# yutongwangBIT/multi_orbslam3

Measured on AMD Instinct MI355X. Metric: tracking+localBA frames/sec (aggregate over agents; 1 agent per GPU), higher is better.
Workload: dtype u8/int32 (ORB front-end, Hamming), f64 (local BA)

## Files before the change

### multi_orbslam3_amd/csrc/lba.hip

```cpp

#include <time.h>

#include <condition_variable>
#include <atomic>
#include <unistd.h>
#include <mutex>
#include <thread>

#include "common.hpp"
#include "wave.hpp"

#include <algorithm>
#include <cmath>
#include <limits>
#include <numeric>
#include <type_traits>

using namespace orbg;

#include "ldlt_mfma.hpp"
#include "ldlt_xcd.hpp"
#include "se3.hpp"
#include "lm_driver.hpp"

// ... 20 lines not shown
struct HostRec { double chi2, scale, maxdiag, chi2_init; int ok; unsigned seq; unsigned long long c_chi2, c_scale, c_ok; };
__host__ __device__ inline unsigned long long rec_tag(unsigned seq) { return (0x9E3779B97F4A7C15ull * ((unsigned long long)seq + 1ull)) | 1ull; }

template <class CamT>
__global__ __launch_bounds__(256) void k_export(int n_edges, int n_poses, int n_points, const lba_edge* __restrict__ edges,
                                               const PoseQ* __restrict__ poses, const double* __restrict__ points, CamT cam,
                                               const double* __restrict__ chi2, uint8_t* __restrict__ out_flags,
                                               double* __restrict__ out_chi2, PoseQ* __restrict__ out_poses,
                                               double* __restrict__ out_points) {
  const int k = blockIdx.x * 256 + threadIdx.x;
  if (k < n_edges) {
    const lba_edge e = edges[k];
    const bool depth_pos = edge_depth_positive(poses[e.pose], points + 3 * (size_t)e.point, cam, e);
    const double thr = e.ur < 0 ? 5.991 : 7.815;
    const double c = chi2[k];
    const bool outlier = c > thr || !depth_pos;
    out_flags[k] = (uint8_t)((depth_pos ? 1 : 0) | (outlier ? 2 : 0));
    if (out_chi2) out_chi2[k] = c;
  }
  if (k < n_poses) out_poses[k] = poses[k];
  if (k < 3 * n_points) out_points[k] = points[k];
}

struct LmIn { double cur_chi, lambda; const double* chi_p; const double* lambda_p; double* lambda_next; };

__device__ __forceinline__ void publish_trial_tail(int n_edge_blocks, const double* __restrict__ partial, unsigned* __restrict__ ticket,
                                                   const double* __restrict__ scale_partial, int n_scale_partial,
                                                   const int* __restrict__ ok_flag, HostRec* __restrict__ rec, unsigned seq, const LmIn lm,
                                                   int ok_override = 1) {
  __shared__ double parts[1024];
  const int np = n_edge_blocks;
  const int tot = min(np + n_scale_partial, 1024);
  for (int i = threadIdx.x; i < tot; i += 256)
    parts[i] = __hip_atomic_load(i < np ? &partial[i] : &scale_partial[i - np], __ATOMIC_RELAXED, __HIP_MEMORY_SCOPE_AGENT);
  __syncthreads();
  if (threadIdx.x == 0) {
    auto ordered_sum = [&](int first, int count) {
      double acc = 0;
      int i = 0;
      for (; i + 16 <= count; i += 16) {
        double v[16];
#pragma unroll
        for (int u = 0; u < 16; u++) v[u] = parts[first + i + u];
#pragma unroll
        for (int u = 0; u < 16; u++) acc += v[u];
      }
      for (; i < count; i++) acc += parts[first + i];
      return acc;
    };
    const int np_l = min(np, 1024), ns_l = max(min(np + n_scale_partial, 1024) - np_l, 0);
    double chi = ordered_sum(0, np_l), scale = ordered_sum(np_l, ns_l);
    for (int i = np_l; i < np; i++) chi += __hip_atomic_load(&partial[i], __ATOMIC_RELAXED, __HIP_MEMORY_SCOPE_AGENT);
    for (int i = ns_l; i < n_scale_partial; i++) scale += __hip_atomic_load(&scale_partial[i], __ATOMIC_RELAXED, __HIP_MEMORY_SCOPE_AGENT);
    const int okv = ok_override != 1 ? ok_override : ok_flag ? *ok_flag : 1;
    {
      const unsigned long long tg = rec_tag(seq), bc = (unsigned long long)__double_as_longlong(chi), bs = (unsigned long long)__double_as_longlong(scale);
      unsigned long long* r64 = reinterpret_cast<unsigned long long*>(rec);
      __hip_atomic_store(r64 + 0, bc, __ATOMIC_RELAXED, __HIP_MEMORY_SCOPE_SYSTEM);
      __hip_atomic_store(r64 + 1, bs, __ATOMIC_RELAXED, __HIP_MEMORY_SCOPE_SYSTEM);
      __hip_atomic_store(&rec->ok, okv, __ATOMIC_RELAXED, __HIP_MEMORY_SCOPE_SYSTEM);
      __hip_atomic_store(&rec->c_chi2, bc ^ tg, __ATOMIC_RELAXED, __HIP_MEMORY_SCOPE_SYSTEM);
      __hip_atomic_store(&rec->c_scale, bs ^ tg, __ATOMIC_RELAXED, __HIP_MEMORY_SCOPE_SYSTEM);
      __hip_atomic_store(&rec->c_ok, (unsigned long long)(unsigned)okv ^ tg, __ATOMIC_RELAXED, __HIP_MEMORY_SCOPE_SYSTEM);
    }
    if (lm.lambda_next) {
      const double cur = lm.chi_p ? *lm.chi_p : lm.cur_chi;
      const double lam = lm.lambda_p ? *lm.lambda_p : lm.lambda;
      const double tempChi = okv ? chi : 1.7976931348623157e308;
      double rho = cur - tempChi;
      rho /= scale + 1e-3;
      const double c3 = 2 * rho - 1;
      double alpha = 1. - c3 * c3 * c3;
      alpha = fmin(alpha, 2. / 3.);
      *lm.lambda_next = lam * fmax(1. / 3., alpha);
    }
    *ticket = 0;
    __hip_atomic_store(&rec->seq, seq, __ATOMIC_RELAXED, __HIP_MEMORY_SCOPE_SYSTEM);
  }
}
__device__ __forceinline__ unsigned trial_arrive(unsigned* __restrict__ ticket) {
  __builtin_amdgcn_fence(__ATOMIC_RELEASE, "agent");
  asm volatile("s_waitcnt vmcnt(0)" ::: "memory");
  return __hip_atomic_fetch_add(ticket, 1u, __ATOMIC_RELAXED, __HIP_MEMORY_SCOPE_AGENT);
}
__device__ __forceinline__ void publish_trial_record(int n_edge_blocks, const double* __restrict__ partial, unsigned* __restrict__ ticket,
                                                     const double* __restrict__ scale_partial, int n_scale_partial,
                                                     const int* __restrict__ ok_flag, HostRec* __restrict__ rec, unsigned seq,
                                                     const LmIn lm = LmIn{0, 0, nullptr, nullptr, nullptr}) {
  __shared__ int s_last;
  if (threadIdx.x == 0) s_last = (trial_arrive(ticket) == (unsigned)n_edge_blocks - 1);
  __syncthreads();
  if (!s_last) return;
  if (threadIdx.x == 0) {
    __builtin_amdgcn_fence(__ATOMIC_ACQUIRE, "agent");
    asm volatile("s_waitcnt vmcnt(0)" ::: "memory");
  }
  __syncthreads();
  publish_trial_tail(n_edge_blocks, partial, ticket, scale_partial, n_scale_partial, ok_flag, rec, seq, lm);
}
constexpr int kOkPublishTimedOut = -3;
__device__ __forceinline__ void publish_trial_when_all_arrived(int n_edge_blocks, const double* __restrict__ partial, unsigned* __restrict__ ticket,
                                                               const double* __restrict__ scale_partial, int n_scale_partial,
                                                               const int* __restrict__ ok_flag, HostRec* __restrict__ rec, unsigned seq, const LmIn lm) {
  __shared__ int s_ok;
  if (threadIdx.x == 0) {
    const long long t0 = (long long)wall_clock64();
    int ok = 1;
    for (unsigned polls = 0;; polls++) {
      if (__hip_atomic_load(ticket, __ATOMIC_RELAXED, __HIP_MEMORY_SCOPE_AGENT) >= (unsigned)n_edge_blocks) break;
      __builtin_amdgcn_s_sleep(1);
      if ((polls & 1023u) == 1023u && (long long)wall_clock64() - t0 > 200000000ll) { ok = kOkPublishTimedOut; break; }
    }
    s_ok = ok;
  }
  __syncthreads();
  publish_trial_tail(n_edge_blocks, partial, ticket, scale_partial, n_scale_partial, ok_flag, rec, seq, lm, s_ok);
}

template <class CamT>
__device__ __forceinline__ double errors_block(int bid, int n_edge_blocks, int n_edges, const lba_edge* __restrict__ edges,
                                               const PoseQ* __restrict__ poses, const double* __restrict__ points, CamT cam, Huber hb,
                                               double* __restrict__ err, double* __restrict__ chi2, double* __restrict__ partial,
                                               int final_mode, unsigned* __restrict__ ticket, const double* __restrict__ scale_partial,
                                               int n_scale_partial, const int* __restrict__ ok_flag, HostRec* __restrict__ rec,
                                               unsigned seq) {
  __shared__ double red[256];
  const int k = bid * 256 + threadIdx.x;
  double c_out = 0;
  double rho0 = 0;
  if (k < n_edges) {
    const lba_edge e = edges[k];
    double er[3], Xc[3];
    edge_error(poses[e.pose], points + 3 * (size_t)e.point, cam, e, er, Xc);
    const double om = (double)e.inv_sigma2;
    const int D = e.ur < 0 ? 2 : 3;
    double c = 0;
    for (int i = 0; i < D; i++) c += er[i] * (om * er[i]);
    err[3 * (size_t)k] = er[0]; err[3 * (size_t)k + 1] = er[1]; err[3 * (size_t)k + 2] = er[2];
    chi2[k] = c;
// ... 180 lines not shown
#pragma unroll
        for (int i = 0; i < 18; i++) out[i] = 0.0;
      } else if (pose_col[e.pose] >= 0 && point_col[e.point] >= 0) {
        for (int k2 = k + 1; k2 < n_edges; k2++) {
          const lba_edge e2 = edges[k2];
          if (e2.pose != e.pose || e2.point != e.point) break;
          double H2[18];
          edge_hpl<FUSED>(T, X, c, hb, e2, k2, err, chi2, H2);
#pragma unroll
          for (int i = 0; i < 18; i++) out[i] += H2[i];
        }
      }
    }
  }
  __syncthreads();
  const int valid = min(256, n_edges - bid * 256);
  double* dst = EB + (size_t)bid * 256 * kEB;
  for (int i = threadIdx.x; i < valid * kEB; i += 256) dst[i] = stage[i];
}
template <bool FUSED, class CamT>
__device__ __forceinline__ void lin_poses_block(int bid, const int* __restrict__ ps_start, const int* __restrict__ ps_edges,
                                                  const lba_edge* __restrict__ edges, const PoseQ* __restrict__ poses,
                                                  const double* __restrict__ points, CamT c, Huber hb, const double* __restrict__ err,
                                                  const double* __restrict__ chi2, double* __restrict__ Hpp, double* __restrict__ bp) {
  __shared__ double wpart[4][27];
  const int p = bid;
  const int b = ps_start[p], e_end = ps_start[p + 1];
  double acc[27];
#pragma unroll
  for (int i = 0; i < 27; i++) acc[i] = 0;
  constexpr int kCh = 3;
  for (int j0 = b + threadIdx.x; j0 < e_end; j0 += 256 * kCh) {
    int kk[kCh];
#pragma unroll
    for (int u = 0; u < kCh; u++) kk[u] = ps_edges[min(j0 + 256 * u, e_end - 1)];
    lba_edge ev[kCh];
#pragma unroll
    for (int u = 0; u < kCh; u++) ev[u] = edges[kk[u]];
    double Xv[kCh][3];
#pragma unroll
    for (int u = 0; u < kCh; u++) {
      const double* Xp = points + 3 * (size_t)ev[u].point;
      Xv[u][0] = Xp[0]; Xv[u][1] = Xp[1]; Xv[u][2] = Xp[2];
    }
    const PoseQ T = poses[ev[0].pose];
#pragma unroll
    for (int u = 0; u < kCh; u++) {
// ... 36 lines not shown
          acc[o++] += h;
        }
#pragma unroll
      for (int a = 0; a < 6; a++) {
        double sacc = 0;
#pragma unroll
        for (int i = 0; i < 3; i++) sacc += B[6 * i + a] * omega_r[i];
        acc[o++] += sacc;
      }
    }
  }
  const int lane = threadIdx.x & 63, wave = threadIdx.x >> 6;
#pragma unroll
  for (int i = 0; i < 27; i++) {
    const double v = wave_sum_f64(acc[i]);
    if (lane == 0) wpart[wave][i] = v;
  }
  __syncthreads();
  if (threadIdx.x < 27) {
    const double v = ((wpart[0][threadIdx.x] + wpart[1][threadIdx.x]) + wpart[2][threadIdx.x]) + wpart[3][threadIdx.x];
    if (threadIdx.x < 21) Hpp[21 * (size_t)p + threadIdx.x] = v;
    else bp[6 * (size_t)p + threadIdx.x - 21] = v;
  }
}


__device__ __forceinline__ double quad_get(double v, int src ) {
  int lo, hi;
  if (src == 1) { lo = __builtin_amdgcn_update_dpp(0, __double2loint(v), 0x55, 0xF, 0xF, true); hi = __builtin_amdgcn_update_dpp(0, __double2hiint(v), 0x55, 0xF, 0xF, true); }
  else if (src == 2) { lo = __builtin_amdgcn_update_dpp(0, __double2loint(v), 0xAA, 0xF, 0xF, true); hi = __builtin_amdgcn_update_dpp(0, __double2hiint(v), 0xAA, 0xF, 0xF, true); }
  else { lo = __builtin_amdgcn_update_dpp(0, __double2loint(v), 0xFF, 0xF, 0xF, true); hi = __builtin_amdgcn_update_dpp(0, __double2hiint(v), 0xFF, 0xF, 0xF, true); }
  return __hiloint2double(hi, lo);
}
template <class CamT>
__device__ __forceinline__ void lin_points_block(int bid, int nL, const int* __restrict__ pt_start, const int* __restrict__ pt_edges,
                                                   const lba_edge* __restrict__ edges, const PoseQ* __restrict__ poses,
                                                   const double* __restrict__ points, CamT c, Huber hb, double* __restrict__ Hll,
                                                   double* __restrict__ bl) {
  const int t = bid * 256 + threadIdx.x;
  const int l = min(t >> 2, nL - 1), q = t & 3;
  const bool mine = (t >> 2) < nL;
  double acc[9];
#pragma unroll
  for (int i = 0; i < 9; i++) acc[i] = 0;
  const int jb = pt_start[l], je = pt_start[l + 1];
  for (int j0 = jb + q; j0 < je; j0 += 8) {
    int id[2];
#pragma unroll
    for (int u = 0; u < 2; u++) id[u] = pt_edges[min(j0 + 4 * u, je - 1)];
    lba_edge ev[2];
#pragma unroll
    for (int u = 0; u < 2; u++) ev[u] = edges[id[u]];
    PoseQ Tv[2];
#pragma unroll
    for (int u = 0; u < 2; u++) Tv[u] = poses[ev[u].pose];
    const double* X = points + 3 * (size_t)ev[0].point;
    const double Xl[3] = {X[0], X[1], X[2]};
#pragma unroll
    for (int u = 0; u < 2; u++)
      if (j0 + 4 * u < je) {
        const lba_edge e = ev[u];
// ... 20 lines not shown
        for (int a = 0; a < 3; a++)
#pragma unroll
          for (int b2 = a; b2 < 3; b2++) {
            double h = 0;
#pragma unroll
            for (int i = 0; i < 3; i++) h += A[3 * i + a] * wom * A[3 * i + b2];
            acc[o++] += h;
          }
#pragma unroll
        for (int a = 0; a < 3; a++) {
          double sacc = 0;
#pragma unroll
          for (int i = 0; i < 3; i++) sacc += A[3 * i + a] * omega_r[i];
          acc[o++] += sacc;
        }
      }
  }
#pragma unroll
  for (int i = 0; i < 9; i++) acc[i] = ((acc[i] + quad_get(acc[i], 1)) + quad_get(acc[i], 2)) + quad_get(acc[i], 3);
  if (mine && q == 0) {
    for (int i = 0; i < 6; i++) Hll[6 * (size_t)l + i] = acc[i];
    for (int i = 0; i < 3; i++) bl[3 * (size_t)l + i] = acc[6 + i];
  }
}
__host__ __device__ inline int errlin_point_blocks(int nL) { return (4 * nL + 255) / 256; }
__host__ __device__ inline int errlin_tail_blocks(int nL) { return errlin_point_blocks(nL) + 1; }

template <class CamT>
__global__ __launch_bounds__(256) void k_lin_all(int nP, int n_edges, const lba_edge* __restrict__ edges, const PoseQ* __restrict__ poses,
                                                const double* __restrict__ points, CamT c, Huber hb, const double* __restrict__ err,
                                                const double* __restrict__ chi2, const int* __restrict__ pose_col,
                                                const int* __restrict__ point_col, double* __restrict__ EB,
                                                const int* __restrict__ ps_start, const int* __restrict__ ps_edges,
                                                double* __restrict__ Hpp, double* __restrict__ bp) {
  if ((int)blockIdx.x < nP) lin_poses_block<false>(blockIdx.x, ps_start, ps_edges, edges, poses, points, c, hb, err, chi2, Hpp, bp);
  else linearize_block<false>(blockIdx.x - nP, n_edges, edges, poses, points, c, hb, const_cast<double*>(err), const_cast<double*>(chi2),
                              pose_col, point_col, EB, TrialPublish{nullptr, nullptr, nullptr, 0, nullptr, nullptr, 0u, 0, LmIn{0, 0, nullptr, nullptr, nullptr}});
}

template <class CamT>
__global__ __launch_bounds__(256) void k_errlin(int nP, int n_edges, const lba_edge* __restrict__ edges, const PoseQ* __restrict__ poses,
                                               const double* __restrict__ points, CamT c, Huber hb, double* __restrict__ err,
                                               double* __restrict__ chi2, const int* __restrict__ pose_col,
                                               const int* __restrict__ point_col, double* __restrict__ EB,
                                               const int* __restrict__ ps_start, const int* __restrict__ ps_edges,
                                               double* __restrict__ Hpp, double* __restrict__ bp, double* __restrict__ partial,
                                               unsigned* __restrict__ ticket, const double* __restrict__ scale_partial, int n_scale_partial,
                                               const int* __restrict__ ok_flag, HostRec* __restrict__ rec, unsigned seq, int n_edge_blocks,
                                               int nL, const int* __restrict__ pt_start, const int* __restrict__ pt_edges,
                                               double* __restrict__ Hll, double* __restrict__ bl, LmIn lm) {
  const int bid = (int)blockIdx.x;
  LBA_PROF_BEGIN(0);
  if (bid < nP) {
    lin_poses_block<true>(bid, ps_start, ps_edges, edges, poses, points, c, hb, err, chi2, Hpp, bp);
  } else if (bid < nP + n_edge_blocks) {
    linearize_block<true>(bid - nP, n_edges, edges, poses, points, c, hb, err, chi2, pose_col, point_col, EB,
                          TrialPublish{partial, ticket, scale_partial, n_scale_partial, ok_flag, rec, seq, n_edge_blocks, lm});
  } else if (bid - nP - n_edge_blocks < errlin_point_blocks(nL)) {
    lin_points_block(bid - nP - n_edge_blocks, nL, pt_start, pt_edges, edges, poses, points, c, hb, Hll, bl);
  } else {
    publish_trial_when_all_arrived(n_edge_blocks, partial, ticket, scale_partial, n_scale_partial, ok_flag, rec, seq, lm);
  }
  LBA_PROF_END();
}


__global__ __launch_bounds__(256) void k_reduce_points(int nL, const int* __restrict__ pt_start, const int* __restrict__ pt_edges,
                                                      const double* __restrict__ EB, double* __restrict__ Hll, double* __restrict__ bl) {
  const int l = blockIdx.x * 256 + threadIdx.x;
  if (l >= nL) return;
  double acc[9];
#pragma unroll
  for (int i = 0; i < 9; i++) acc[i] = 0;
  const int jb = pt_start[l], je = pt_start[l + 1];
  double part[4][9];
#pragma unroll
  for (int q = 0; q < 4; q++)
#pragma unroll
    for (int i = 0; i < 9; i++) part[q][i] = 0;
  for (int j0 = jb; j0 < je; j0 += 4) {
    int id[4];
#pragma unroll
    for (int q = 0; q < 4; q++) id[q] = pt_edges[min(j0 + q, je - 1)];
    double v[4][9];
// ... 167 lines not shown
                                               const int* __restrict__ ok_flag, HostRec* __restrict__ rec, unsigned seq, int n_edge_blocks,
                                               int nL, const int* __restrict__ pt_start, const int* __restrict__ pt_edges,
                                               double* __restrict__ Hll, double* __restrict__ bl, LmIn lm) {
  int bid = (int)blockIdx.x;
  if (bid >= n_errlin_blocks) {
    bid -= n_errlin_blocks;
    if (bid < n_sort_blocks) { sort_pf_block<256, kPrep256Cap>(bid, nL, pf_start, pf_edges_w, pf_col_w, lm_mask, edges, pose_col); return; }
    bid -= n_sort_blocks;
    if (bid < kPrep256Pad) { if (St) ldltm::image_pad_range(n_unknowns, St, bid * 256 + (int)threadIdx.x, kPrep256Pad * 256); return; }
    bid -= kPrep256Pad;
    for (int i = bid * 256 + (int)threadIdx.x; i < n_zero; i += kPrep256Zero * 256) xzero[i] = 0.0;
    return;
  }

  
  if (bid < nP) {
    lin_poses_block<true>(bid, ps_start, ps_edges, edges, poses, points, c, hb, err, chi2, Hpp, bp);
  } else if (bid < nP + n_edge_blocks) {
    linearize_block<true>(bid - nP, n_edges, edges, poses, points, c, hb, err, chi2, pose_col, point_col, EB,
                          TrialPublish{partial, ticket, scale_partial, n_scale_partial, ok_flag, rec, seq, n_edge_blocks, lm});
  } else if (bid - nP - n_edge_blocks < errlin_point_blocks(nL)) {
    lin_points_block(bid - nP - n_edge_blocks, nL, pt_start, pt_edges, edges, poses, points, c, hb, Hll, bl);
  } else {
    publish_trial_when_all_arrived(n_edge_blocks, partial, ticket, scale_partial, n_scale_partial, ok_flag, rec, seq, lm);
  }
}

__global__ __launch_bounds__(kSortPfThreads) void k_prep(int n_sort_blocks, int nL, const int* __restrict__ pf_start, int* __restrict__ pf_edges,
                                                        int* __restrict__ pf_col, unsigned long long* __restrict__ lm_mask,
                                                        const lba_edge* __restrict__ edges, const int* __restrict__ pose_col,
                                                        int n, double* __restrict__ St, double* __restrict__ xzero, int n_zero) {
  constexpr int kPadBlocks = 32;
  const int bid = (int)blockIdx.x;
  if (bid < n_sort_blocks) { sort_pf_block<kSortPfThreads, kSortPfCap>(bid, nL, pf_start, pf_edges, pf_col, lm_mask, edges, pose_col); return; }
  if (bid < n_sort_blocks + kPadBlocks) {
    if (St) ldltm::image_pad_range(n, St, (bid - n_sort_blocks) * kSortPfThreads + (int)threadIdx.x, kPadBlocks * kSortPfThreads);
    return;
  }
  const int nz = (int)gridDim.x - n_sort_blocks - kPadBlocks;
  for (int i = (bid - n_sort_blocks - kPadBlocks) * kSortPfThreads + (int)threadIdx.x; i < n_zero; i += nz * kSortPfThreads) xzero[i] = 0.0;
}

__device__ __forceinline__ void build_items_block(int pr, int nP, int nL, const unsigned long long* __restrict__ lm_mask,
                                                  const int* __restrict__ pf_start, const int* __restrict__ pf_edges,
                                                  const int* __restrict__ pf_col, PairItem* __restrict__ items, int cap,
                                                  int* __restrict__ pair_count) {
  __shared__ int wcount[4];
// ... 327 lines not shown
};
struct lba_handle {
  int device = 0;
  hipStream_t stream = nullptr;
  bool ext_stream = false;
  LdltSolver ldlt;
  long long xcd_timeouts = 0;
  DevBuf<lba_edge> d_edges;
  PinnedBuf<lba_edge> edges_pin;
  DevBuf<PairItem> d_items_dev;
  DevBuf<int> d_pair_count;
  DevBuf<PoseQ> d_poses[2];
  DevBuf<double> d_points[2];
  DevBuf<double> d_err, d_chi2, d_partial, d_bs, d_x;
  LinSet lin[2];
  DevBuf<double> d_lambda0;
  DevBuf<int> d_ok;
  PinnedBuf<HostRec> rec;
  unsigned rec_seq = 0;
  PinnedBuf<uint8_t> up_h, dl_h;
  DevBuf<uint8_t> up_d;
  DevBuf<double> d_scale_partial;
  DevBuf<unsigned> d_ticket;
  StreamSignal sig;
  std::vector<int> s_pose_deg, s_point_deg, s_pose_col, s_point_col, s_pf_deg, s_f1, s_f2, s_f3, s_fill, s_row_off, s_junk;
  std::vector<unsigned> s_cnt4;
  int prof_on = 0;
  hipEvent_t prof_ev[2] = {nullptr, nullptr};
  double prof_sum_ms = 0; long long prof_n = 0; int prof_n_unknowns = 0;
  long long prof_solves = 0;
  std::thread worker;
  std::mutex mu;
  std::condition_variable cv;
  std::atomic<bool> quit{false};
  std::atomic<int> job_state{0};
  const lba_problem* job_p = nullptr; StopRef job_stop; lba_result* job_r = nullptr;
  int job_status = ORBG_OK;
  double job_ms = 0;
};

extern "C" int lba_create(int device, int cap_poses, int cap_points, int cap_edges, lba_handle** out) {
  if (!out || cap_poses < 0 || cap_points < 0 || cap_edges < 0) return ORBG_BAD_ARG;
  int rc = select_device(device);
  if (rc) return rc;
  lba_handle* h = new lba_handle();
  h->device = device;
  h->ldlt.read_env();
  h->ldlt.keep_dense = true;
  if (orbg::create_stream(&h->stream, "lba") != hipSuccess) { delete h; return ORBG_HIP_ERROR; }
  if ((rc = h->rec.reserve(4)) || (rc = h->d_ok.reserve(4))) { delete h; return rc; }
  memset(h->rec.h, 0, 4 * sizeof(HostRec));
  (void)cap_poses; (void)cap_points; (void)cap_edges;
  *out = h;
  return ORBG_OK;
}

extern "C" int lba_set_stream(lba_handle* h, void* hip_stream) {
  if (!h) return ORBG_BAD_ARG;
  if (h->job_state.load() != 0) return ORBG_BAD_ARG;
  int rc = select_device(h->device);
  if (rc) return rc;
  return orbg::swap_stream(&h->stream, &h->ext_stream, hip_stream, "lba");
}

extern "C" int lba_destroy(lba_handle* h) {
  if (!h) return ORBG_BAD_ARG;
  if (h->worker.joinable()) {
    { std::lock_guard<std::mutex> lk(h->mu); h->quit = true; }
    h->cv.notify_all();
    h->worker.join();
  }
  (void)hipSetDevice(h->device);
  (void)hipStreamSynchronize(h->stream);
  h->ldlt.release();
  h->d_edges.release(); h->edges_pin.release(); h->d_items_dev.release(); h->d_pair_count.release();
  for (int i = 0; i < 2; i++) { h->d_poses[i].release(); h->d_points[i].release(); }
  h->d_err.release(); h->d_chi2.release(); h->d_partial.release(); h->d_bs.release(); h->d_x.release();
  for (LinSet& L : h->lin) L.release();
  h->d_lambda0.release(); h->d_ok.release(); h->rec.release();
  h->up_h.release(); h->dl_h.release(); h->up_d.release(); h->d_scale_partial.release(); h->d_ticket.release(); h->sig.release();
  for (auto& e : h->prof_ev) if (e) { (void)hipEventDestroy(e); e = nullptr; }
  if (!h->ext_stream) orbg::release_stream(h->stream);
  delete h;
  return ORBG_OK;
}

struct TraceAcc {
  double t[8] = {0}; long n = 0; const char* name;
  explicit TraceAcc(const char* nm) : name(nm) {}
  ~TraceAcc() {
    if (n && getenv("ORBG_TRACE")) {
      fprintf(stderr, "[orbgpu trace] %s n=%ld:", name, n);
      for (int i = 0; i < 8; i++) fprintf(stderr, " %.1f", t[i] / n * 1e6);
      fprintf(stderr, " us\n");
    }
  }
};
static inline double now_s() { timespec ts; clock_gettime(CLOCK_MONOTONIC, &ts); return ts.tv_sec + 1e-9 * ts.tv_nsec; }

__global__ __launch_bounds__(256) void k_upload16(const uint4* __restrict__ src, uint4* __restrict__ dst, unsigned n16) {
  const unsigned i = blockIdx.x * 256u + threadIdx.x;
  if (i < n16) dst[i] = src[i];
}
static void upload16(const uint8_t* src, uint8_t* dst, size_t bytes, hipStream_t st) {
  const unsigned n16 = (unsigned)((bytes + 15) / 16);
  hipLaunchKernelGGL(k_upload16, dim3((n16 + 255) / 256), dim3(256), 0, st, reinterpret_cast<const uint4*>(src),
                     reinterpret_cast<uint4*>(dst), n16);
}
static int upload_arena(lba_handle* h, size_t off0, size_t off1, hipStream_t st) {
  if (off1 <= off0) return ORBG_OK;
  upload16(h->up_h.d + off0, h->up_d.p + off0, off1 - off0, st);
  ORBG_HIP(hipGetLastError());
  return ORBG_OK;
}

static int lba_solve_attempt(lba_handle* h, const lba_problem* p, StopRef stop_ref, lba_result* r);
static int lba_solve_impl(lba_handle* h, const lba_problem* p, StopRef stop_ref, lba_result* r) {
  bool retried = false;
  const int rc = ldlt_retry(h->ldlt, h->stream, [&] { return lba_solve_attempt(h, p, stop_ref, r); }, &retried);
  if (retried) h->xcd_timeouts++;
  return rc;
}



struct Arena {
  PoseQ* poses; double* points;
  int *pose_col, *point_col, *pt_start, *ps_start, *pf_start;
  int *cur_pt, *cur_ps, *cur_pf;
  int *pt_edges, *ps_edges, *pf_edges, *pf_col;
  unsigned long long* lm_mask;
  int *pair_i1, *pair_i2, *pair_start;
  PairItem* items;
};
// ... 35 lines not shown
};

constexpr int kUpdThreads = 64;

template <class CamT>
struct LbaRun : LbaStructure {
  lba_handle* const h;
  const hipStream_t st;
  const lba_problem* const p;
  lba_result* const r;
  const CamT& cam;
  StopCheck stop;
  LmState lm;
  Huber hb;
  const lba_edge* d_edges = nullptr;
  Arena D{};
  PoseQ* posesB[3] = {};
  double* pointsB[3] = {};
  struct { uint8_t* flags; double* chi2; PoseQ* poses; double* points; } out{};
  size_t o_rflags = 0, o_rchi = 0, o_rposes = 0, o_rpoints = 0;
  int n_blocks_u = 0;
  bool first2 = false;
  bool prof_this_solve = false, prof_pending = false;

  LbaRun(lba_handle* h_, const lba_problem* p_, lba_result* r_, const CamT& cam_, StopRef stop_ref)
      : h(h_), st(h_->stream), p(p_), r(r_), cam(cam_) {
    stop.ref = stop_ref;
    NP = p->n_poses; NX = p->n_points; NE = p->n_edges;
    hb.delta_mono = (float)std::sqrt(5.991); hb.dsqr_mono = hb.delta_mono * hb.delta_mono;
    hb.delta_stereo = (float)std::sqrt(7.815); hb.dsqr_stereo = hb.delta_stereo * hb.delta_stereo;
  }

  void errors(int buf, int final_mode) {
    if (NE > 0)
      hipLaunchKernelGGL(k_errors<CamT>, dim3(n_blocks_e), dim3(256), 0, st, NE, d_edges, posesB[buf], pointsB[buf], cam, hb,
                         h->d_err.p, h->d_chi2.p, h->d_partial.p, final_mode, h->d_ticket.p, h->d_scale_partial.p, n_blocks_u,
                         h->d_ok.p, h->rec.d, final_mode ? ++h->rec_seq : 0u);
  }
  void linearise(int buf, int set) {
    const LinSet& L = h->lin[set];
    if (NE > 0 || nP > 0)
      hipLaunchKernelGGL(k_lin_all<CamT>, dim3(nP + (NE > 0 ? n_blocks_e : 0)), dim3(256), 0, st, nP, NE, d_edges, posesB[buf],
                         pointsB[buf], cam, hb, h->d_err.p, h->d_chi2.p, D.pose_col, D.point_col, L.EB.p, D.ps_start,
                         D.ps_edges, L.Hpp.p, L.bp.p);
    if (nL > 0)
      hipLaunchKernelGGL(k_reduce_points, dim3((nL + 255) / 256), dim3(256), 0, st, nL, D.pt_start, D.pt_edges, L.EB.p, L.Hll.p, L.bl.p);
// ... 233 lines not shown
      for (int k = 0; k < NE; k++) {
        const int lc = A.point_col[edges[k].point], pc = A.pose_col[edges[k].pose];
        A.pt_edges[f1[lc]++] = k;
        if (pc >= 0) {
          A.ps_edges[f2[pc]++] = k;
          if (!kRig || !rig_secondary[k]) A.pf_edges[f3[lc]++] = k;
        }
      }
    }
  }
  void initial_state() {
    for (int i = 0; i < NP; i++) {
      const float* T = p->poses + 16 * (size_t)i;
      const double R[9] = {T[0], T[1], T[2], T[4], T[5], T[6], T[8], T[9], T[10]};
      quat_from_R(R, H.poses[i].q);
      quat_normalize(H.poses[i].q);
      H.poses[i].t[0] = T[3]; H.poses[i].t[1] = T[7]; H.poses[i].t[2] = T[11];
    }
    for (size_t i = 0; i < 3 * (size_t)NX; i++) H.points[i] = p->points[i];
  }

  int buffers() {
    int rc;
    if ((rc = upload_arena(h, 0, off_a, st))) return rc;
    d_edges = h->d_edges.p;
    D = at(h->up_d.p);
    if (dev_lists) { D.pair_i1 = nullptr; D.pair_i2 = nullptr; }
    if (dev_items) {
      D.pair_start = nullptr;
      if ((rc = h->d_items_dev.reserve((size_t)n_pairs_all * item_cap)) || (rc = h->d_pair_count.reserve(std::max(n_pairs_all, 1)))) return rc;
      D.items = h->d_items_dev.p;
    }
    if ((rc = h->d_poses[1].reserve(std::max(NP, 1))) || (rc = h->d_points[1].reserve(std::max<size_t>(3 * (size_t)NX, 1))) ||
        (rc = h->d_poses[0].reserve(std::max(NP, 1))) || (rc = h->d_points[0].reserve(std::max<size_t>(3 * (size_t)NX, 1))) ||
        (rc = h->d_err.reserve(std::max<size_t>(3 * (size_t)NE, 1))) || (rc = h->d_chi2.reserve(std::max(NE, 1))) ||
        (rc = h->d_partial.reserve(std::max(n_blocks_e, 1))) || (rc = h->lin[0].reserve(NE, nL, nP)) ||
        (rc = h->lin[1].reserve(NE, nL, nP)) || (rc = h->d_lambda0.reserve(4)) ||
        (rc = h->d_bs.reserve(std::max(n, 1))) ||
        (rc = h->d_x.reserve(std::max<size_t>((size_t)n + 3 * (size_t)nL, 1))))
      return rc;
    posesB[0] = D.poses; posesB[1] = h->d_poses[1].p; posesB[2] = h->d_poses[0].p;
    pointsB[0] = D.points; pointsB[1] = h->d_points[1].p; pointsB[2] = h->d_points[0].p;
    return ORBG_OK;
  }
  int pick_solver() {
    int rc;
    if ((rc = h->ldlt.plan(n, st))) return rc;
    n_blocks_u = (NP + NX + kUpdThreads - 1) / kUpdThreads;
    if ((rc = h->d_scale_partial.reserve(std::max(n_blocks_u, 1)))) return rc;
    if (!h->d_ticket.p) {
      if ((rc = h->d_ticket.reserve(4))) return rc;
      ORBG_HIP(hipMemsetAsync(h->d_ticket.p, 0, 4 * sizeof(unsigned), st));
    }
    size_t off = 0;
    auto take = [&](size_t bytes) { const size_t o = off; off = (off + bytes + 63) & ~(size_t)63; return o; };
    o_rposes = take(sizeof(PoseQ) * (size_t)NP); o_rpoints = take(24 * (size_t)NX); o_rflags = take((size_t)NE);
    o_rchi = take(r->edge_chi2 ? 8 * (size_t)NE : 0);
    if ((rc = h->dl_h.reserve(off + 64))) return rc;
    out.flags = h->dl_h.d + o_rflags;
    out.chi2 = r->edge_chi2 ? reinterpret_cast<double*>(h->dl_h.d + o_rchi) : (double*)nullptr;
    out.poses = reinterpret_cast<PoseQ*>(h->dl_h.d + o_rposes);
    out.points = reinterpret_cast<double*>(h->dl_h.d + o_rpoints);
    prof_this_solve = h->prof_on && (h->prof_solves++ & 3) == 0;
    return ORBG_OK;
  }

  int first_linearisation() {
    first2 = dev_lists && NE > 0 && nL > 0 && !stop();
    if (first2 || !stop()) {
      const int set = lm.ls ^ 1;
      if (first2) {
        if (dev_csr) {
          hipLaunchKernelGGL(k_csr_fill, dim3(n_blocks_e), dim3(256), 0, st, NE, d_edges, D.pose_col, D.point_col, D.cur_pt, D.cur_ps,
                             D.cur_pf, D.pt_edges, D.ps_edges, D.pf_edges);
          const int n_blocks_l = (nL + 255) / 256;
          hipLaunchKernelGGL(k_csr_sort, dim3(nP + n_blocks_l + kPrep256Pad + kPrep256Zero), dim3(256), 0, st, nP, nL, D.ps_start,
// ... 62 lines not shown
    if (dev_items) {
      if (stop()) return ORBG_OK;
      if (!dev_lists && (rc = upload_arena(h, off_a, o_pair_start, st))) return rc;
      if (nL > 0 && !first2)
        hipLaunchKernelGGL(k_build_items, dim3(n_pairs_all), dim3(256), 0, st, nP, nL, D.lm_mask, D.pf_start, D.pf_edges, D.pf_col,
                           h->d_items_dev.p, item_cap, h->d_pair_count.p);
      ORBG_HIP(hipGetLastError());
      return ORBG_OK;
    }
    for (int i = 0; i < n_pairs_all; i++) A.pair_start[i + 1] += A.pair_start[i];
    std::vector<int>& fill = h->s_fill;
    fill.assign(A.pair_start, A.pair_start + n_pairs_all);
    const std::vector<int>& row_off = h->s_row_off;
    for (int l = 0; l < nL; l++) {
      const int b0 = A.pf_start[l], e0 = A.pf_start[l + 1];
      for (int a2 = b0; a2 < e0; a2++) {
        const int ro = row_off[A.pf_col[a2]], ea = A.pf_edges[a2];
        for (int b2 = a2; b2 < e0; b2++) A.items[fill[ro + A.pf_col[b2]]++] = PairItem{ea, A.pf_edges[b2], l};
      }
    }
    return upload_arena(h, off_a, o_end, st);
  }

  int launch_trial(int trial, bool first_of_spec, bool lambda_on_device, bool round_may_end, bool* speculated) {
    LmState& m = lm;
    int rc;
    const double* lam_p = lambda_on_device ? h->d_lambda0.p : (const double*)nullptr;
    if (!(m.solve_version == m.version - 1 && first_of_spec) && (rc = solve(m.ls, m.lambda, lam_p))) return rc;
    update(m.cur, trial, m.ls, m.lambda, lam_p);
    *speculated = false;
    if (NE == 0) return finish_record(m.ls, m.lambda, 1, 0, true);
    if (!(m.last_round && round_may_end)) {
      const int set = m.ls ^ 1;
      errlin(trial, set, true, LmIn{m.currentChi, m.lambda, lambda_on_device ? h->d_lambda0.p + 2 : (const double*)nullptr, lam_p,
                                    h->d_lambda0.p + 1});
      *speculated = true;
      if (!round_may_end && nP > 0) {
        if ((rc = solve(set, 0.0, h->d_lambda0.p + 1))) return rc;
        m.solve_version = m.version;
      }
      if (round_may_end && !lambda_on_device) {
        finish_lambda_init(set);
        m.fin_version = m.version;
      }
    } else if (!lambda_on_device) {
      errors_export(trial);
      if ((rc = h->sig.post(st))) return rc;
      m.exp_version = m.version; m.exp_buf = trial;
    } else {
      errors(trial, 1);
    }
    ORBG_HIP(hipGetLastError());
    return poll_record();
  }
  int optimize(int iterations, int* done_out) {
    LmState& m = lm;
    int done = 0, rc;
    bool ok = true;
    for (int it = 0; it < iterations && !stop() && ok; it++) {
      const bool used_spec = m.spec_ready;
      if (m.spec_ready) {
        m.ls ^= 1;
        m.spec_ready = false;
      } else {
        if (!m.err_valid) { errors(m.cur, 0); m.err_valid = true; }
        linearise(m.cur, m.ls);
      }
      bool lambda_on_device = false;
      if (it == 0) {
        if (NE > 0) {
          if (!(used_spec && m.fin_version == m.version)) finish_lambda_init(m.ls);
          lambda_on_device = true;
        } else {
          if ((rc = finish_record(m.ls, 0.0, 0, 1, false))) return rc;
          m.currentChi = h->rec.h->chi2;
          m.lambda = lm_lambda_init(p->lambda_init, h->rec.h->maxdiag);
        }
        m.ni = 2; m.nBad = 0;
      }
      if (!lambda_on_device && m.first_chi) { r->chi2_initial = m.currentChi; m.first_chi = false; }
      const bool round_may_end = it + 1 >= iterations || m.nBad >= 2;
      double iniChi = m.currentChi;
      double rho = 0;
      int qmax = 0;
      do {
        const int trial = (m.cur + 1) % 3;
        m.version++;
        bool speculated;
        if ((rc = launch_trial(trial, qmax == 0 && used_spec, lambda_on_device, round_may_end, &speculated))) return rc;
        if (lambda_on_device) {
          m.currentChi = h->rec.h->chi2_init;
          m.lambda = lm_lambda_init(p->lambda_init, h->rec.h->maxdiag);
          lambda_on_device = false;
          if (m.first_chi) { r->chi2_initial = m.currentChi; m.first_chi = false; }
          iniChi = m.currentChi;
        }
        bool accepted;
        rho = lm_trial_verdict(m, h->rec.h->ok != 0, h->rec.h->chi2, h->rec.h->scale, &accepted);
        if (accepted) {
          m.cur = trial;
          m.err_valid = true;
          m.spec_ready = speculated;
        } else {
          m.err_valid = false;
          m.spec_ready = false;
        }
        qmax++;
        stop.trials_done++;
      } while (lm_try_again(rho, qmax < 10, stop()));
      done++;
      r->chi2_final = m.currentChi;
      if (r->trace && r->trace_len < r->trace_cap) {
        r->trace[3 * r->trace_len] = m.lambda; r->trace[3 * r->trace_len + 1] = m.currentChi; r->trace[3 * r->trace_len + 2] = qmax;
        r->trace_len++;
// ... 270 lines not shown
```

Measured before the change: 9018.

## Fold lambda-init max-diagonal reduction into errlin kernel and pre-solve next round

Pose and point linearisation blocks now each post their max Hessian diagonal into a slot and bump a second ticket. The publisher block waits for those arrivals, reduces them, and writes the initial lambda and chi2, so the separate finish_lambda_init launch is skipped. When the round is about to end it also speculatively launches the next round's first solve using the on-device lambda. Tickets are now cleared inside the upload kernel instead of by a one-time memset. The changes remove a kernel launch and a host round-trip per LM round, at the cost of extra polling in the publisher block and more complex synchronisation.

Measured after the change: 9046, median of 5. Within noise of the previous version (+0.3%).

```diff
diff --git a/multi_orbslam3_amd/csrc/lba.hip b/multi_orbslam3_amd/csrc/lba.hip
--- a/multi_orbslam3_amd/csrc/lba.hip
+++ b/multi_orbslam3_amd/csrc/lba.hip
@@ -66,9 +66,20 @@
   if (k < 3 * n_points) out_points[k] = points[k];
 }
 
-struct LmIn { double cur_chi, lambda; const double* chi_p; const double* lambda_p; double* lambda_next; };
-
-__device__ __forceinline__ void publish_trial_tail(int n_edge_blocks, const double* __restrict__ partial, unsigned* __restrict__ ticket,
+constexpr int kOkPublishTimedOut = -3;
+struct LmIn {
+  double cur_chi, lambda; const double* chi_p; const double* lambda_p; double* lambda_next;
+  int finish_init; double lambda_init; double* lambda0; double* diag_part;
+};
+constexpr int kTicketWords = 4;
+
+__device__ __forceinline__ void post_and_arrive(double* __restrict__ slot, double v, unsigned* __restrict__ ticket) {
+  __hip_atomic_store(slot, v, __ATOMIC_RELAXED, __HIP_MEMORY_SCOPE_AGENT);
+  asm volatile("s_waitcnt vmcnt(0)" ::: "memory");
+  __hip_atomic_fetch_add(ticket, 1u, __ATOMIC_RELAXED, __HIP_MEMORY_SCOPE_AGENT);
+}
+
+__device__ __forceinline__ double publish_trial_tail(int n_edge_blocks, const double* __restrict__ partial, unsigned* __restrict__ ticket,
                                                    const double* __restrict__ scale_partial, int n_scale_partial,
                                                    const int* __restrict__ ok_flag, HostRec* __restrict__ rec, unsigned seq, const LmIn lm,
                                                    int ok_override = 1) {
@@ -78,6 +89,7 @@
   for (int i = threadIdx.x; i < tot; i += 256)
     parts[i] = __hip_atomic_load(i < np ? &partial[i] : &scale_partial[i - np], __ATOMIC_RELAXED, __HIP_MEMORY_SCOPE_AGENT);
   __syncthreads();
+  double chi_out = 0;
   if (threadIdx.x == 0) {
     auto ordered_sum = [&](int first, int count) {
       double acc = 0;
@@ -96,6 +108,7 @@
     double chi = ordered_sum(0, np_l), scale = ordered_sum(np_l, ns_l);
     for (int i = np_l; i < np; i++) chi += __hip_atomic_load(&partial[i], __ATOMIC_RELAXED, __HIP_MEMORY_SCOPE_AGENT);
     for (int i = ns_l; i < n_scale_partial; i++) scale += __hip_atomic_load(&scale_partial[i], __ATOMIC_RELAXED, __HIP_MEMORY_SCOPE_AGENT);
+    chi_out = chi;
     const int okv = ok_override != 1 ? ok_override : ok_flag ? *ok_flag : 1;
     {
       const unsigned long long tg = rec_tag(seq), bc = (unsigned long long)__double_as_longlong(chi), bs = (unsigned long long)__double_as_longlong(scale);
@@ -118,9 +131,10 @@
       alpha = fmin(alpha, 2. / 3.);
       *lm.lambda_next = lam * fmax(1. / 3., alpha);
     }
-    *ticket = 0;
+    if (ok_override != kOkPublishTimedOut) *ticket = 0;
     __hip_atomic_store(&rec->seq, seq, __ATOMIC_RELAXED, __HIP_MEMORY_SCOPE_SYSTEM);
   }
+  return chi_out;
 }
 __device__ __forceinline__ unsigned trial_arrive(unsigned* __restrict__ ticket) {
   __builtin_amdgcn_fence(__ATOMIC_RELEASE, "agent");
@@ -142,23 +156,49 @@
   __syncthreads();
   publish_trial_tail(n_edge_blocks, partial, ticket, scale_partial, n_scale_partial, ok_flag, rec, seq, lm);
 }
-constexpr int kOkPublishTimedOut = -3;
 __device__ __forceinline__ void publish_trial_when_all_arrived(int n_edge_blocks, const double* __restrict__ partial, unsigned* __restrict__ ticket,
                                                                const double* __restrict__ scale_partial, int n_scale_partial,
-                                                               const int* __restrict__ ok_flag, HostRec* __restrict__ rec, unsigned seq, const LmIn lm) {
+                                                               const int* __restrict__ ok_flag, HostRec* __restrict__ rec, unsigned seq, const LmIn lm,
+                                                               int n_diag) {
   __shared__ int s_ok;
+  const long long t0 = (long long)wall_clock64();
+  auto wait_arrivals = [&](const unsigned* tk, unsigned want) {
+    for (unsigned polls = 0;; polls++) {
+      if (__hip_atomic_load(tk, __ATOMIC_RELAXED, __HIP_MEMORY_SCOPE_AGENT) >= want) return 1;
+      __builtin_amdgcn_s_sleep(1);
+      if ((polls & 1023u) == 1023u && (long long)wall_clock64() - t0 > 200000000ll) return kOkPublishTimedOut;
+    }
+  };
+  if (threadIdx.x == 0) s_ok = wait_arrivals(ticket, (unsigned)n_edge_blocks);
+  __syncthreads();
+  const double chi = publish_trial_tail(n_edge_blocks, partial, ticket, scale_partial, n_scale_partial, ok_flag, rec, seq, lm, s_ok);
+  if (!lm.finish_init) return;
+  __shared__ double red_d[256];
+  __shared__ int s_ok2;
+  __syncthreads();
+  if (threadIdx.x == 0) s_ok2 = s_ok == 1 ? wait_arrivals(ticket + 1, (unsigned)n_diag) : s_ok;
+  __syncthreads();
+  const bool arrived = s_ok2 == 1;
+  double mx = 0;
+  if (arrived)
+    for (int i = threadIdx.x; i < n_diag; i += 256)
+      mx = fmax(mx, __hip_atomic_load(&lm.diag_part[i], __ATOMIC_RELAXED, __HIP_MEMORY_SCOPE_AGENT));
+  red_d[threadIdx.x] = mx;
+  __syncthreads();
+  for (int s = 128; s > 0; s >>= 1) {
+    if ((int)threadIdx.x < s) red_d[threadIdx.x] = fmax(red_d[threadIdx.x], red_d[threadIdx.x + s]);
+    __syncthreads();
+  }
   if (threadIdx.x == 0) {
-    const long long t0 = (long long)wall_clock64();
-    int ok = 1;
-    for (unsigned polls = 0;; polls++) {
-      if (__hip_atomic_load(ticket, __ATOMIC_RELAXED, __HIP_MEMORY_SCOPE_AGENT) >= (unsigned)n_edge_blocks) break;
-      __builtin_amdgcn_s_sleep(1);
-      if ((polls & 1023u) == 1023u && (long long)wall_clock64() - t0 > 200000000ll) { ok = kOkPublishTimedOut; break; }
-    }
-    s_ok = ok;
-  }
-  __syncthreads();
-  publish_trial_tail(n_edge_blocks, partial, ticket, scale_partial, n_scale_partial, ok_flag, rec, seq, lm, s_ok);
+    if (arrived) {
+      rec->chi2_init = chi; rec->maxdiag = red_d[0];
+      lm.lambda0[0] = lm.lambda_init > 0 ? lm.lambda_init : 1e-5 * red_d[0];
+      lm.lambda0[2] = chi;
+      ticket[1] = 0;
+    } else {
+      rec->chi2_init = chi; rec->maxdiag = __longlong_as_double(0x7FF8000000000000ll);
+    }
+  }
 }
 
 template <class CamT>
@@ -385,7 +425,8 @@
 __device__ __forceinline__ void lin_poses_block(int bid, const int* __restrict__ ps_start, const int* __restrict__ ps_edges,
                                                   const lba_edge* __restrict__ edges, const PoseQ* __restrict__ poses,
                                                   const double* __restrict__ points, CamT c, Huber hb, const double* __restrict__ err,
-                                                  const double* __restrict__ chi2, double* __restrict__ Hpp, double* __restrict__ bp) {
+                                                  const double* __restrict__ chi2, double* __restrict__ Hpp, double* __restrict__ bp,
+                                                  double* __restrict__ diag_slot = nullptr, unsigned* __restrict__ diag_ticket = nullptr) {
   __shared__ double wpart[4][27];
   const int p = bid;
   const int b = ps_start[p], e_end = ps_start[p + 1];
@@ -468,6 +509,15 @@
     if (threadIdx.x < 21) Hpp[21 * (size_t)p + threadIdx.x] = v;
     else bp[6 * (size_t)p + threadIdx.x - 21] = v;
   }
+  if (diag_slot && threadIdx.x == 0) {
+    double mx = 0;
+#pragma unroll
+    for (int j = 0; j < 6; j++) {
+      const int d = j == 0 ? 0 : j == 1 ? 6 : j == 2 ? 11 : j == 3 ? 15 : j == 4 ? 18 : 20;
+      mx = fmax(mx, fabs(((wpart[0][d] + wpart[1][d]) + wpart[2][d]) + wpart[3][d]));
+    }
+    post_and_arrive(diag_slot, mx, diag_ticket);
+  }
 }
 
 
@@ -482,7 +532,8 @@
 __device__ __forceinline__ void lin_points_block(int bid, int nL, const int* __restrict__ pt_start, const int* __restrict__ pt_edges,
                                                    const lba_edge* __restrict__ edges, const PoseQ* __restrict__ poses,
                                                    const double* __restrict__ points, CamT c, Huber hb, double* __restrict__ Hll,
-                                                   double* __restrict__ bl) {
+                                                   double* __restrict__ bl, double* __restrict__ diag_slot = nullptr,
+                                                   unsigned* __restrict__ diag_ticket = nullptr) {
   const int t = bid * 256 + threadIdx.x;
   const int l = min(t >> 2, nL - 1), q = t & 3;
   const bool mine = (t >> 2) < nL;
@@ -549,6 +600,15 @@
     for (int i = 0; i < 6; i++) Hll[6 * (size_t)l + i] = acc[i];
     for (int i = 0; i < 3; i++) bl[3 * (size_t)l + i] = acc[6 + i];
   }
+  if (diag_slot) {
+    __shared__ double wmax[4];
+    double mx = (mine && q == 0) ? fmax(fabs(acc[0]), fmax(fabs(acc[3]), fabs(acc[5]))) : 0.0;
+#pragma unroll
+    for (int o = 32; o > 0; o >>= 1) mx = fmax(mx, __shfl_xor(mx, o, 64));
+    if ((threadIdx.x & 63) == 0) wmax[threadIdx.x >> 6] = mx;
+    __syncthreads();
+    if (threadIdx.x == 0) post_and_arrive(diag_slot, fmax(fmax(wmax[0], wmax[1]), fmax(wmax[2], wmax[3])), diag_ticket);
+  }
 }
 __host__ __device__ inline int errlin_point_blocks(int nL) { return (4 * nL + 255) / 256; }
 __host__ __device__ inline int errlin_tail_blocks(int nL) { return errlin_point_blocks(nL) + 1; }
@@ -578,15 +638,19 @@
                                                double* __restrict__ Hll, double* __restrict__ bl, LmIn lm) {
   const int bid = (int)blockIdx.x;
   LBA_PROF_BEGIN(0);
+  const int pb = bid - nP - n_edge_blocks;
   if (bid < nP) {
-    lin_poses_block<true>(bid, ps_start, ps_edges, edges, poses, points, c, hb, err, chi2, Hpp, bp);
+    lin_poses_block<true>(bid, ps_start, ps_edges, edges, poses, points, c, hb, err, chi2, Hpp, bp,
+                          lm.finish_init ? lm.diag_part + bid : nullptr, ticket + 1);
   } else if (bid < nP + n_edge_blocks) {
     linearize_block<true>(bid - nP, n_edges, edges, poses, points, c, hb, err, chi2, pose_col, point_col, EB,
                           TrialPublish{partial, ticket, scale_partial, n_scale_partial, ok_flag, rec, seq, n_edge_blocks, lm});
-  } else if (bid - nP - n_edge_blocks < errlin_point_blocks(nL)) {
-    lin_points_block(bid - nP - n_edge_blocks, nL, pt_start, pt_edges, edges, poses, points, c, hb, Hll, bl);
+  } else if (pb < errlin_point_blocks(nL)) {
+    lin_points_block(pb, nL, pt_start, pt_edges, edges, poses, points, c, hb, Hll, bl, lm.finish_init ? lm.diag_part + nP + pb : nullptr,
+                     ticket + 1);
   } else {
-    publish_trial_when_all_arrived(n_edge_blocks, partial, ticket, scale_partial, n_scale_partial, ok_flag, rec, seq, lm);
+    publish_trial_when_all_arrived(n_edge_blocks, partial, ticket, scale_partial, n_scale_partial, ok_flag, rec, seq, lm,
+                                   nP + errlin_point_blocks(nL));
   }
   LBA_PROF_END();
 }
@@ -800,7 +864,7 @@
   } else if (bid - nP - n_edge_blocks < errlin_point_blocks(nL)) {
     lin_points_block(bid - nP - n_edge_blocks, nL, pt_start, pt_edges, edges, poses, points, c, hb, Hll, bl);
   } else {
-    publish_trial_when_all_arrived(n_edge_blocks, partial, ticket, scale_partial, n_scale_partial, ok_flag, rec, seq, lm);
+    publish_trial_when_all_arrived(n_edge_blocks, partial, ticket, scale_partial, n_scale_partial, ok_flag, rec, seq, lm, 0);
   }
 }
 
@@ -1174,6 +1238,7 @@
   DevBuf<uint8_t> up_d;
   DevBuf<double> d_scale_partial;
   DevBuf<unsigned> d_ticket;
+  DevBuf<double> d_diag_part;
   StreamSignal sig;
   std::vector<int> s_pose_deg, s_point_deg, s_pose_col, s_point_col, s_pf_deg, s_f1, s_f2, s_f3, s_fill, s_row_off, s_junk;
   std::vector<unsigned> s_cnt4;
@@ -1200,7 +1265,7 @@
   h->ldlt.read_env();
   h->ldlt.keep_dense = true;
   if (orbg::create_stream(&h->stream, "lba") != hipSuccess) { delete h; return ORBG_HIP_ERROR; }
-  if ((rc = h->rec.reserve(4)) || (rc = h->d_ok.reserve(4))) { delete h; return rc; }
+  if ((rc = h->rec.reserve(4)) || (rc = h->d_ok.reserve(4)) || (rc = h->d_ticket.reserve(kTicketWords))) { delete h; return rc; }
   memset(h->rec.h, 0, 4 * sizeof(HostRec));
   (void)cap_poses; (void)cap_points; (void)cap_edges;
   *out = h;
@@ -1230,7 +1295,7 @@
   h->d_err.release(); h->d_chi2.release(); h->d_partial.release(); h->d_bs.release(); h->d_x.release();
   for (LinSet& L : h->lin) L.release();
   h->d_lambda0.release(); h->d_ok.release(); h->rec.release();
-  h->up_h.release(); h->dl_h.release(); h->up_d.release(); h->d_scale_partial.release(); h->d_ticket.release(); h->sig.release();
+  h->up_h.release(); h->dl_h.release(); h->up_d.release(); h->d_scale_partial.release(); h->d_ticket.release(); h->d_diag_part.release(); h->sig.release();
   for (auto& e : h->prof_ev) if (e) { (void)hipEventDestroy(e); e = nullptr; }
   if (!h->ext_stream) orbg::release_stream(h->stream);
   delete h;
@@ -1250,18 +1315,21 @@
 };
 static inline double now_s() { timespec ts; clock_gettime(CLOCK_MONOTONIC, &ts); return ts.tv_sec + 1e-9 * ts.tv_nsec; }
 
-__global__ __launch_bounds__(256) void k_upload16(const uint4* __restrict__ src, uint4* __restrict__ dst, unsigned n16) {
+__global__ __launch_bounds__(256) void k_upload16(const uint4* __restrict__ src, uint4* __restrict__ dst, unsigned n16,
+                                                 unsigned* __restrict__ clear_tickets) {
   const unsigned i = blockIdx.x * 256u + threadIdx.x;
   if (i < n16) dst[i] = src[i];
-}
-static void upload16(const uint8_t* src, uint8_t* dst, size_t bytes, hipStream_t st) {
+  if (clear_tickets && blockIdx.x == gridDim.x - 1 && threadIdx.x == 255)
+    for (int w = 0; w < kTicketWords; w++) clear_tickets[w] = 0u;
+}
+static void upload16(const uint8_t* src, uint8_t* dst, size_t bytes, hipStream_t st, unsigned* clear_tickets = nullptr) {
   const unsigned n16 = (unsigned)((bytes + 15) / 16);
-  hipLaunchKernelGGL(k_upload16, dim3((n16 + 255) / 256), dim3(256), 0, st, reinterpret_cast<const uint4*>(src),
-                     reinterpret_cast<uint4*>(dst), n16);
-}
-static int upload_arena(lba_handle* h, size_t off0, size_t off1, hipStream_t st) {
-  if (off1 <= off0) return ORBG_OK;
-  upload16(h->up_h.d + off0, h->up_d.p + off0, off1 - off0, st);
+  hipLaunchKernelGGL(k_upload16, dim3(std::max(1u, (n16 + 255) / 256)), dim3(256), 0, st, reinterpret_cast<const uint4*>(src),
+                     reinterpret_cast<uint4*>(dst), n16, clear_tickets);
+}
+static int upload_arena(lba_handle* h, size_t off0, size_t off1, hipStream_t st, unsigned* clear_tickets = nullptr) {
+  if (off1 <= off0 && !clear_tickets) return ORBG_OK;
+  upload16(h->up_h.d + off0, h->up_d.p + off0, off1 > off0 ? off1 - off0 : 0, st, clear_tickets);
   ORBG_HIP(hipGetLastError());
   return ORBG_OK;
 }
@@ -1343,6 +1411,7 @@
   int n_blocks_u = 0;
   bool first2 = false;
   bool prof_this_solve = false, prof_pending = false;
+  const bool finish_kernel = [] { const char* e = getenv("ORBG_LBA_FINISH_KERNEL"); return e && e[0] == '1'; }();
 
   LbaRun(lba_handle* h_, const lba_problem* p_, lba_result* r_, const CamT& cam_, StopRef stop_ref)
       : h(h_), st(h_->stream), p(p_), r(r_), cam(cam_) {
@@ -1622,7 +1691,7 @@
 
   int buffers() {
     int rc;
-    if ((rc = upload_arena(h, 0, off_a, st))) return rc;
+    if ((rc = upload_arena(h, 0, off_a, st, h->d_ticket.p))) return rc;
     d_edges = h->d_edges.p;
     D = at(h->up_d.p);
     if (dev_lists) { D.pair_i1 = nullptr; D.pair_i2 = nullptr; }
@@ -1636,6 +1705,7 @@
         (rc = h->d_err.reserve(std::max<size_t>(3 * (size_t)NE, 1))) || (rc = h->d_chi2.reserve(std::max(NE, 1))) ||
         (rc = h->d_partial.reserve(std::max(n_blocks_e, 1))) || (rc = h->lin[0].reserve(NE, nL, nP)) ||
         (rc = h->lin[1].reserve(NE, nL, nP)) || (rc = h->d_lambda0.reserve(4)) ||
+        (rc = h->d_diag_part.reserve(std::max(nP + errlin_point_blocks(nL), 1))) ||
         (rc = h->d_bs.reserve(std::max(n, 1))) ||
         (rc = h->d_x.reserve(std::max<size_t>((size_t)n + 3 * (size_t)nL, 1))))
       return rc;
@@ -1648,10 +1718,6 @@
     if ((rc = h->ldlt.plan(n, st))) return rc;
     n_blocks_u = (NP + NX + kUpdThreads - 1) / kUpdThreads;
     if ((rc = h->d_scale_partial.reserve(std::max(n_blocks_u, 1)))) return rc;
-    if (!h->d_ticket.p) {
-      if ((rc = h->d_ticket.reserve(4))) return rc;
-      ORBG_HIP(hipMemsetAsync(h->d_ticket.p, 0, 4 * sizeof(unsigned), st));
-    }
     size_t off = 0;
     auto take = [&](size_t bytes) { const size_t o = off; off = (off + bytes + 63) & ~(size_t)63; return o; };
     o_rposes = take(sizeof(PoseQ) * (size_t)NP); o_rpoints = take(24 * (size_t)NX); o_rflags = take((size_t)NE);
@@ -1760,7 +1826,7 @@
     return upload_arena(h, off_a, o_end, st);
   }
 
-  int launch_trial(int trial, bool first_of_spec, bool lambda_on_device, bool round_may_end, bool* speculated) {
+  int launch_trial(int trial, bool first_of_spec, bool lambda_on_device, bool round_may_end, bool round_ends_if_accepted, bool* speculated) {
     LmState& m = lm;
     int rc;
     const double* lam_p = lambda_on_device ? h->d_lambda0.p : (const double*)nullptr;
@@ -1770,16 +1836,22 @@
     if (NE == 0) return finish_record(m.ls, m.lambda, 1, 0, true);
     if (!(m.last_round && round_may_end)) {
       const int set = m.ls ^ 1;
+      const bool init_next = round_may_end && !lambda_on_device;
+      const bool fold = init_next && !finish_kernel;
       errlin(trial, set, true, LmIn{m.currentChi, m.lambda, lambda_on_device ? h->d_lambda0.p + 2 : (const double*)nullptr, lam_p,
-                                    h->d_lambda0.p + 1});
+                                    h->d_lambda0.p + 1, fold ? 1 : 0, p->lambda_init, h->d_lambda0.p, h->d_diag_part.p});
       *speculated = true;
       if (!round_may_end && nP > 0) {
         if ((rc = solve(set, 0.0, h->d_lambda0.p + 1))) return rc;
         m.solve_version = m.version;
       }
-      if (round_may_end && !lambda_on_device) {
-        finish_lambda_init(set);
+      if (init_next) {
+        if (!fold) finish_lambda_init(set);
         m.fin_version = m.version;
+        if (round_ends_if_accepted && !m.last_round && nP > 0 && !finish_kernel) {
+          if ((rc = solve(set, 0.0, h->d_lambda0.p))) return rc;
+          m.solve_version = m.version;
+        }
       }
     } else if (!lambda_on_device) {
       errors_export(trial);
@@ -1805,9 +1877,10 @@
         linearise(m.cur, m.ls);
       }
       bool lambda_on_device = false;
+      const bool fin_valid = used_spec && m.fin_version == m.version;
       if (it == 0) {
         if (NE > 0) {
-          if (!(used_spec && m.fin_version == m.version)) finish_lambda_init(m.ls);
+          if (!fin_valid) finish_lambda_init(m.ls);
           lambda_on_device = true;
         } else {
           if ((rc = finish_record(m.ls, 0.0, 0, 1, false))) return rc;
@@ -1825,9 +1898,12 @@
         const int trial = (m.cur + 1) % 3;
         m.version++;
         bool speculated;
-        if ((rc = launch_trial(trial, qmax == 0 && used_spec, lambda_on_device, round_may_end, &speculated))) return rc;
+        if ((rc = launch_trial(trial, qmax == 0 && used_spec && (it > 0 || fin_valid), lambda_on_device, round_may_end,
+                               it + 1 >= iterations, &speculated)))
+          return rc;
         if (lambda_on_device) {
           m.currentChi = h->rec.h->chi2_init;
+          if (h->rec.h->maxdiag != h->rec.h->maxdiag) return ORBG_INTERNAL;
           m.lambda = lm_lambda_init(p->lambda_init, h->rec.h->maxdiag);
           lambda_on_device = false;
           if (m.first_chi) { r->chi2_initial = m.currentChi; m.first_chi = false; }
```
